# ybubnov/libhuffman

Measured on AMD Instinct MI355X. Metric: encode+decode GiB/s (uncompressed) on 64KiB blocks, higher is better.
Workload: dtype u8; 1 GPU; configs[2]: 1 GiB Zipf-distributed bytes (zipf255 seed 3), blocksize=64KiB; generator=zipf255, bytes_per_gpu=1073741824, blocksize=65536, blocks_per_gpu=16384, compressed_bytes_per_gpu=1006904592, parallelism=block-sharded x1, bit_exact_roundtrip=True, decoder=sub-index (verified), one table pass per symbol

## Files before the change

### libhuffman_amd/csrc/host/ctx.hpp

```cpp
#pragma once

#include "workspace.hpp"

struct hufgpu_ctx {
    int device;
    hipStream_t stream;
    char err[512];

    uint64_t ws_blocks;
    uint32_t *d_hist;
    hufcode_t *d_codetab;
    int16_t *d_treebuf;
    HufBlockMeta *d_meta;
    uint64_t *d_offsets;
    TwoLevel enc_sizes;
    uint64_t ws_chunks;
    uint32_t *d_chunk_hist;
    uint64_t *d_chunk_tot, *d_chunk_bits;

    uint64_t dws_blocks;
    HufDecodeMeta *d_dmeta;
    uint64_t *d_out_offsets;
    int32_t *d_status;
    TwoLevel dec_lens;
    uint32_t *d_fix_count;
    uint32_t *d_fix_blocks;
    uint32_t *d_fix_flag;

    uint64_t disc_wgs, disc_cands;
    uint32_t *d_wg_counts;
    void *d_disc_slots;
    uint64_t *d_disc_masks;
    uint64_t *d_wg_base;
    uint64_t *d_cand, *d_cand_end, *d_chain;
    int32_t *d_cand_status;
    uint32_t *d_nxt;
    uint64_t *d_walk;
    uint64_t *d_spec_off;

    uint64_t big_lanes, big_sub_bytes;
    uint64_t *d_big_entry, *d_big_exit, *d_big_pre, *d_big_wgpre, *d_big_wgscratch, *d_big_first_pos, *d_big_first_g, *d_big_last_pos;
    uint32_t *d_big_cnt;
    void *d_big_sub;
    uint64_t *d_big_offs;

    uint64_t fixed_ws;
    uint64_t *d_result;
    uint64_t complete_used, complete_raw;
    uint64_t *h_result;
    uint64_t *d_zipf;

    int profiling;
    int prof_used;
    int cur_slot;
    int n_stages;
    hipEvent_t (*ev)[MAX_STAGES + 1];
    int slot_stages[PROF_SLOTS];
    int slot_kind[PROF_SLOTS];
    int decode_pending;
    hipStream_t last_stream;
    const uint8_t *last_st;
    const uint64_t *last_offsets;
    uint8_t *last_out;
    uint64_t last_stream_len, last_out_cap, last_nblocks;
    uint64_t last_failing;
    int last_max_tree;

    uint64_t *h_bstage, *d_bstage;
    uint64_t bstage_words;
    hipEvent_t bstage_ev;
    int bstage_pending;
    uint64_t bws_blocks, bws_items;
    uint64_t *d_bprefix, *d_bobase, *d_bzero;
    uint32_t *d_blk_item;
    unsigned long long *d_item_fail;
    uint64_t *d_item_res, *h_item_res;
    uint64_t *d_bitem_offs;

    uint64_t rws_blocks, rws_ranges;
    unsigned long long *d_rcover;
    uint64_t *d_rrel, *d_rplan;
    uint32_t *d_rflag;
    unsigned long long *d_rcounters;
    unsigned long long *d_rtpairs;
    uint64_t rcounters[8];
    uint8_t *d_rscratch;
    uint64_t rscratch_bytes;

    uint64_t gws_blocks, gws_parts;
    uint32_t *d_gcnt, *d_glist;
    TwoLevel gat_scan;
    uint64_t *d_gtotal;
    void *d_gparts;
    int cus;

    uint64_t fws_words, fws_tiles, fws_edge_tiles;
    uint32_t *d_fbitmap, *d_ftcnt;
    TwoLevel find_scan;
    uint8_t *d_fedges;
    uint64_t frws_words, frws_tiles;
    uint32_t *d_frdbits, *d_frrbits, *d_frdcnt, *d_frrcnt;
    TwoLevel frec_scan;
    uint64_t *d_frdtotal;
    uint64_t fsel_ws;
    uint64_t *d_fsel_first;

    uint64_t sbws_blocks, sbws_chunks;
    uint32_t *d_sb_state;
    uint64_t *d_sb_pay, *d_sb_chunk_tot, *d_sb_chunk_bits;
    unsigned long long *d_sb_unbuilt;

    uint64_t uws_blocks, uws_pieces;
    uint32_t *d_urow_of, *d_urow_blk, *d_upiece;
    uint64_t *d_upairs, *d_unew;
    unsigned long long *d_ucount;
};

static char g_err[512] = "";

static void set_err(hufgpu_ctx *ctx, const char *fmt, ...)
{
    char buf[512];
    va_list ap;
    va_start(ap, fmt);
    vsnprintf(buf, sizeof(buf), fmt, ap);
    va_end(ap);
    snprintf(g_err, sizeof(g_err), "%s", buf);
    if (ctx) snprintf(ctx->err, sizeof(ctx->err), "%s", buf);
    fprintf(stderr, "libhuffman(gpu): %s\n", buf);
}

#define HIP_OK(ctx, call)                                                                   \
    do {                                                                                    \
        hipError_t e_ = (call);                                                             \
        if (e_ != hipSuccess) {                                                             \
            set_err((ctx), "%s failed: %s (%s:%d)", #call, hipGetErrorString(e_), __FILE__, \
                    __LINE__);                                                              \
            return HUFE_FATAL;                                                              \
        }                                                                                   \
    } while (0)


static hipError_t g_ws_error = hipSuccess;
static int ws_hip(hipError_t e)
{
    if (e == hipSuccess) return 0;
    g_ws_error = e;
    (void)hipGetLastError();
    return 1;
}
static int ws_hip_alloc_device(void **p, uint64_t bytes) { return ws_hip(hipMalloc(p, bytes)); }
static int ws_hip_alloc_pinned(void **p, uint64_t bytes) { return ws_hip(hipHostMalloc(p, bytes, hipHostMallocDefault)); }
static void ws_hip_free_device(void *p) { (void)hipFree(p); }
static void ws_hip_free_pinned(void *p) { (void)hipHostFree(p); }
static int ws_hip_zero_device(void *p, uint64_t bytes) { return ws_hip(hipMemset(p, 0, bytes)); }
static int ws_hip_wait(void) { return ws_hip(hipDeviceSynchronize()); }
static const ws_hooks WS_HIP = {ws_hip_alloc_device, ws_hip_alloc_pinned, ws_hip_free_device, ws_hip_free_pinned,
                                ws_hip_zero_device, ws_hip_wait};

#define WS_ROW(type, member, flags, expr) \
    {offsetof(type, member), [](uint64_t n, uint64_t m) -> uint64_t { (void)n; (void)m; return (expr); }, flags}
#define DEV(member, expr) WS_ROW(hufgpu_ctx, member, 0, expr)
#define DEV0(member, expr) WS_ROW(hufgpu_ctx, member, WS_ZERO, expr)
#define PIN(member, expr) WS_ROW(hufgpu_ctx, member, WS_PINNED, expr)
#define SCAN_GROUPS(n) ((n) / SCAN_GROUP + 2)

static const ws_buf WS_SCAN[] = {
    WS_ROW(TwoLevel, vals, 0, n * sizeof(uint64_t)),
    WS_ROW(TwoLevel, local, 0, n * sizeof(uint64_t)),
    WS_ROW(TwoLevel, gsum, 0, SCAN_GROUPS(n) * sizeof(uint64_t)),
    WS_ROW(TwoLevel, gprefix, 0, SCAN_GROUPS(n) * sizeof(uint64_t)),
    WS_ROW(TwoLevel, gcount, WS_ZERO, SCAN_GROUPS(n) * SCAN_TICKET_STRIDE * sizeof(uint32_t)),
    WS_ROW(TwoLevel, done, WS_ZERO, sizeof(uint32_t)),
};
static const ws_buf WS_FIXED[] = {
    DEV(d_result, 8 * sizeof(uint64_t)), PIN(h_result, 16 * sizeof(uint64_t)), DEV(d_walk, DISC_WORDS * sizeof(uint64_t)),
    DEV(d_zipf, 255 * sizeof(uint64_t)), DEV(d_big_offs, (SPEC_WORDS + 2) * sizeof(uint64_t)),
    DEV(d_rcounters, 8 * sizeof(unsigned long long)), DEV(d_gtotal, sizeof(uint64_t)),
    DEV(d_ucount, UPD_WORDS * sizeof(unsigned long long)), DEV(d_sb_unbuilt, sizeof(unsigned long long)),
};
static const ws_buf WS_ENCODE[] = {
    DEV(d_hist, n * HUF_NSYM * sizeof(uint64_t)),
    DEV(d_codetab, n * HUF_NSYM * sizeof(hufcode_t)), DEV(d_treebuf, n * HUF_TREE_STRIDE * sizeof(int16_t)),
    DEV(d_meta, n * sizeof(HufBlockMeta)), DEV(d_offsets, (n + 1) * sizeof(uint64_t)),
};
static const ws_buf WS_CHUNK[] = {
    DEV(d_chunk_hist, n * HUF_NSYM * sizeof(uint32_t)), DEV(d_chunk_tot, n * sizeof(uint64_t)), DEV(d_chunk_bits, n * sizeof(uint64_t)),
};
static const ws_buf WS_DECODE[] = {
    DEV(d_dmeta, n * sizeof(HufDecodeMeta)), DEV(d_out_offsets, (n + 1) * sizeof(uint64_t)), DEV(d_status, n * sizeof(int32_t)),
    DEV0(d_fix_count, 2 * sizeof(uint32_t)), DEV(d_fix_blocks, n * sizeof(uint32_t)), DEV0(d_fix_flag, n * sizeof(uint32_t)),
    DEV(dec_lens.gmin, SCAN_GROUPS(n) * sizeof(uint64_t)),
};
#define DISC_GCAP(n) (((n) + DISC_SCAN_GROUP - 1) / DISC_SCAN_GROUP + 1)
static const ws_buf WS_DISC_WGS[] = {
    DEV(d_wg_counts, n * sizeof(uint32_t)),
    DEV(d_wg_base, (n + 1 + 2 * DISC_GCAP(n)) * sizeof(uint64_t)),
    DEV(d_disc_masks, n * DISC_THREADS * sizeof(uint64_t)), DEV(d_disc_slots, n * DISC_SLOTS * sizeof(DiscSlot)),
};
static const ws_buf WS_DISC_CANDS[] = {
    DEV(d_cand, n * sizeof(uint64_t)), DEV(d_cand_end, n * sizeof(uint64_t)), DEV(d_chain, (n + 1) * sizeof(uint64_t)),
    DEV(d_cand_status, n * sizeof(int32_t)), DEV(d_nxt, n * sizeof(uint32_t)), DEV(d_spec_off, (n + 1) * sizeof(uint64_t)),
};
static const ws_buf WS_BIG_LANES[] = {
    DEV(d_big_entry, n * sizeof(uint64_t)), DEV(d_big_exit, n * sizeof(uint64_t)), DEV(d_big_pre, (n + 1) * sizeof(uint64_t)),
    DEV(d_big_wgpre, (n / DEC_THREADS + 4) * sizeof(uint64_t)), DEV(d_big_wgscratch, (n / DEC_THREADS + 4) * sizeof(uint64_t)),
    DEV(d_big_first_pos, n * sizeof(uint64_t)), DEV(d_big_first_g, n * sizeof(uint64_t)), DEV(d_big_last_pos, n * sizeof(uint64_t)),
    DEV(d_big_cnt, n * sizeof(uint32_t)),
};
static const ws_buf WS_BIG_SUB[] = {DEV(d_big_sub, n)};
static const ws_buf WS_BSTAGE[] = {PIN(h_bstage, n * sizeof(uint64_t)), DEV(d_bstage, n * sizeof(uint64_t))};
static const ws_buf WS_BATCH[] = {
    DEV(d_bprefix, (n + 1) * sizeof(uint64_t)), DEV(d_bobase, n * sizeof(uint64_t)), DEV0(d_bzero, SCAN_GROUPS(n) * sizeof(uint64_t)),
    DEV(d_blk_item, n * sizeof(uint32_t)), DEV(d_item_fail, m * sizeof(unsigned long long)), DEV(d_item_res, 3 * m * sizeof(uint64_t)),
    DEV(d_bitem_offs, (m + 1) * sizeof(uint64_t)), PIN(h_item_res, 3 * m * sizeof(uint64_t)),
};
static const ws_buf WS_RANGE[] = {
    DEV(d_rcover, n * sizeof(unsigned long long)), DEV(d_rrel, n * sizeof(uint64_t)), DEV(d_rtpairs, n * sizeof(unsigned long long)),
    DEV(d_rplan, 4 * m * sizeof(uint64_t)), DEV(d_rflag, m * sizeof(uint32_t)),
};
static const ws_buf WS_RSCRATCH[] = {DEV(d_rscratch, n)};
static const ws_buf WS_GATHER_BLOCKS[] = {DEV(d_gcnt, 2 * n * sizeof(uint32_t)), DEV(d_glist, n * sizeof(uint32_t))};
static const ws_buf WS_GATHER_PARTS[] = {DEV(d_gparts, n * sizeof(GatherPart))};
static const ws_buf WS_FIND_WORDS[] = {DEV(d_fbitmap, n * sizeof(uint32_t))};
static const ws_buf WS_FIND_TILES[] = {DEV(d_ftcnt, n * sizeof(uint32_t))};
static const ws_buf WS_FIND_EDGES[] = {DEV(d_fedges, n * FIND_EDGE_SLOT)};
static const ws_buf WS_FIND_REC_WORDS[] = {DEV(d_frdbits, n * sizeof(uint32_t)), DEV(d_frrbits, n * sizeof(uint32_t))};
static const ws_buf WS_FIND_REC_TILES[] = {DEV(d_frdcnt, n * sizeof(uint32_t)), DEV(d_frrcnt, n * sizeof(uint32_t)), DEV(d_frdtotal, sizeof(uint64_t))};
static const ws_buf WS_FIND_SEL[] = {DEV(d_fsel_first, n * sizeof(uint64_t))};
static const ws_buf WS_SB_BLOCKS[] = {DEV(d_sb_state, n * sizeof(uint32_t)), DEV(d_sb_pay, n * sizeof(uint64_t))};
static const ws_buf WS_SB_CHUNKS[] = {DEV(d_sb_chunk_tot, n * sizeof(uint64_t)), DEV(d_sb_chunk_bits, n * sizeof(uint64_t))};
static const ws_buf WS_UPD_BLOCKS[] = {
    DEV(d_urow_of, n * sizeof(uint32_t)), DEV(d_urow_blk, n * sizeof(uint32_t)), DEV(d_upairs, 2 * n * sizeof(uint64_t)),
    DEV(d_unew, (n + 1) * sizeof(uint64_t)),
};
static const ws_buf WS_UPD_PIECES[] = {DEV(d_upiece, n * sizeof(uint32_t))};

enum { G_FIXED, G_ENCODE, G_CHUNK, G_DECODE, G_DISC_WGS, G_DISC_CANDS, G_BIG_LANES, G_BIG_SUB, G_BSTAGE, G_BATCH, G_RANGE,
       G_RSCRATCH, G_GATHER_BLOCKS, G_GATHER_PARTS, G_FIND_WORDS, G_FIND_TILES, G_FIND_EDGES, G_FIND_REC_WORDS, G_FIND_REC_TILES, G_FIND_SEL, G_SB_BLOCKS, G_SB_CHUNKS, G_UPD_BLOCKS,
       G_UPD_PIECES, G_COUNT };
#define ROWS(a) a, (int)(sizeof(a) / sizeof(a[0]))
#define CAP(member) {offsetof(hufgpu_ctx, member), WS_NO_CAP}
#define CAPS(m0, m1) {offsetof(hufgpu_ctx, m0), offsetof(hufgpu_ctx, m1)}
#define NO_SCAN NULL, 0, 0
#define SCAN_AT(member) ROWS(WS_SCAN), offsetof(hufgpu_ctx, member)
static const ws_group WS[G_COUNT] = {
    {"fixed", ROWS(WS_FIXED), CAP(fixed_ws), WS_EXACT, false, NO_SCAN},
    {"encode", ROWS(WS_ENCODE), CAP(ws_blocks), WS_EIGHTH, false, SCAN_AT(enc_sizes)},
    {"encode chunks", ROWS(WS_CHUNK), CAP(ws_chunks), WS_EIGHTH, false, NO_SCAN},
    {"decode", ROWS(WS_DECODE), CAP(dws_blocks), WS_EIGHTH, false, SCAN_AT(dec_lens)},
    {"discovery workgroups", ROWS(WS_DISC_WGS), CAP(disc_wgs), WS_EIGHTH, false, NO_SCAN},
    {"discovery candidates", ROWS(WS_DISC_CANDS), CAP(disc_cands), WS_EIGHTH, false, NO_SCAN},
    {"big-block lanes", ROWS(WS_BIG_LANES), CAP(big_lanes), WS_EIGHTH, true, NO_SCAN},
    {"big-block sub-index", ROWS(WS_BIG_SUB), CAP(big_sub_bytes), WS_EXACT, true, NO_SCAN},
    {"batch staging", ROWS(WS_BSTAGE), CAP(bstage_words), WS_QUARTER, false, NO_SCAN},
    {"batch", ROWS(WS_BATCH), CAPS(bws_blocks, bws_items), WS_EIGHTH, false, NO_SCAN},
    {"ranges", ROWS(WS_RANGE), CAPS(rws_blocks, rws_ranges), WS_EIGHTH, false, NO_SCAN},
    {"range scratch", ROWS(WS_RSCRATCH), CAP(rscratch_bytes), WS_EXACT, true, NO_SCAN},
    {"gather blocks", ROWS(WS_GATHER_BLOCKS), CAP(gws_blocks), WS_DOUBLE, false, SCAN_AT(gat_scan)},
    {"gather parts", ROWS(WS_GATHER_PARTS), CAP(gws_parts), WS_DOUBLE, false, NO_SCAN},
    {"find words", ROWS(WS_FIND_WORDS), CAP(fws_words), WS_DOUBLE, false, NO_SCAN},
    {"find tiles", ROWS(WS_FIND_TILES), CAP(fws_tiles), WS_DOUBLE, false, SCAN_AT(find_scan)},
    {"find edges", ROWS(WS_FIND_EDGES), CAP(fws_edge_tiles), WS_DOUBLE, false, NO_SCAN},
    {"find record words", ROWS(WS_FIND_REC_WORDS), CAP(frws_words), WS_DOUBLE, false, NO_SCAN},
    {"find record tiles", ROWS(WS_FIND_REC_TILES), CAP(frws_tiles), WS_DOUBLE, false, SCAN_AT(frec_scan)},
    {"find select", ROWS(WS_FIND_SEL), CAP(fsel_ws), WS_EXACT, false, NO_SCAN},
    {"sub-build blocks", ROWS(WS_SB_BLOCKS), CAP(sbws_blocks), WS_EIGHTH, false, NO_SCAN},
    {"sub-build chunks", ROWS(WS_SB_CHUNKS), CAP(sbws_chunks), WS_EIGHTH, false, NO_SCAN},
    {"update blocks", ROWS(WS_UPD_BLOCKS), CAP(uws_blocks), WS_EIGHTH, false, NO_SCAN},
    {"update pieces", ROWS(WS_UPD_PIECES), CAP(uws_pieces), WS_EIGHTH, false, NO_SCAN},
};

static int grow_ws(hufgpu_ctx *c, int group, uint64_t need0, uint64_t need1 = 0)
{
    if (ws_grow(&WS_HIP, c, &WS[group], need0, need1) == 0) return HUFE_OK;
    if (WS[group].soft) return HUFE_MEMORY;
    set_err(c, "no workspace for %s (%llu, %llu): %s", WS[group].name, (unsigned long long)need0, (unsigned long long)need1,
            hipGetErrorString(g_ws_error));
    return HUFE_FATAL;
}
static int grow_ws2(hufgpu_ctx *c, int g0, uint64_t need0, int g1, uint64_t need1)
{
    const int rc = grow_ws(c, g0, need0);
    return rc ? rc : grow_ws(c, g1, need1);
}

static int ensure_encode_ws(hufgpu_ctx *c, uint64_t nblocks)
{
    const bool grows = nblocks > c->ws_blocks;
    const int rc = grow_ws(c, G_ENCODE, nblocks);
    if (grows) ws_release(&WS_HIP, c, &WS[G_CHUNK]);
    return rc;
}
static int ensure_chunk_ws(hufgpu_ctx *c, uint64_t nchunks) { return grow_ws(c, G_CHUNK, nchunks); }
static int ensure_decode_ws(hufgpu_ctx *c, uint64_t nblocks) { return grow_ws(c, G_DECODE, nblocks); }
static int ensure_batch_ws(hufgpu_ctx *c, uint64_t nblocks, uint64_t nitems) { return grow_ws(c, G_BATCH, nblocks, nitems); }
static int ensure_range_ws(hufgpu_ctx *c, uint64_t nblocks, uint64_t nranges) { return grow_ws(c, G_RANGE, nblocks, nranges); }
static int ensure_gather_ws(hufgpu_ctx *c, uint64_t nblocks, uint64_t nparts) { return grow_ws2(c, G_GATHER_BLOCKS, nblocks, G_GATHER_PARTS, nparts); }
static int ensure_find_ws(hufgpu_ctx *c, uint64_t nwords, uint64_t ntiles) { return grow_ws2(c, G_FIND_WORDS, nwords, G_FIND_TILES, ntiles); }
static int ensure_update_ws(hufgpu_ctx *c, uint64_t nblocks, uint64_t npieces) { return grow_ws2(c, G_UPD_BLOCKS, nblocks, G_UPD_PIECES, npieces); }
static int ensure_sub_build_ws(hufgpu_ctx *c, uint64_t nblocks, uint64_t nchunks) { return grow_ws2(c, G_SB_BLOCKS, nblocks, G_SB_CHUNKS, nchunks); }

static int grow_range_scratch(hufgpu_ctx *ctx, uint64_t bytes)
{
    if (bytes <= ctx->rscratch_bytes) return HUFE_OK;
    if (bytes > ((uint64_t)1 << 46)) {
        (void)ws_hip_wait();
        ws_release(&WS_HIP, ctx, &WS[G_RSCRATCH]);
        return HUFE_MEMORY;
    }
    if (grow_ws(ctx, G_RSCRATCH, bytes + bytes / 8) == HUFE_OK) return HUFE_OK;
    return grow_ws(ctx, G_RSCRATCH, bytes);
}

static void free_batch_stage(hufgpu_ctx *c)
{
    if (c->bstage_pending) (void)hipEventSynchronize(c->bstage_ev);
    ws_release(&WS_HIP, c, &WS[G_BSTAGE]);
    c->bstage_pending = 0;
}

extern "C" int hufgpu_device_count(void)
{
    int n = 0;
    if (hipGetDeviceCount(&n) != hipSuccess) {
        (void)hipGetLastError();
        return 0;
    }
    int usable = 0;
    for (int d = 0; d < n; d++) {
        hipDeviceProp_t p;
        if (hipGetDeviceProperties(&p, d) == hipSuccess && strncmp(p.gcnArchName, "gfx950", 6) == 0) usable++;
    }
    return usable;
}

extern "C" const char *hufgpu_last_error(const hufgpu_ctx_t *ctx) { return ctx ? ctx->err : g_err; }

static int ctx_init(hufgpu_ctx *ctx)
{
    HIP_OK(NULL, hipSetDevice(ctx->device));
    const int rc = grow_ws(ctx, G_FIXED, 1);
    if (rc) return rc;
    uint64_t cum[255], acc = 0;
    for (int r = 1; r <= 255; r++) {
        acc += (1ull << 32) / (uint64_t)r;
        cum[r - 1] = acc;
    }
    HIP_OK(ctx, hipMemcpy(ctx->d_zipf, cum, sizeof(cum), hipMemcpyHostToDevice));
    return HUFE_OK;
}

extern "C" int hufgpu_ctx_create(hufgpu_ctx_t **out, int device)
{
    if (!out) return HUFE_ARGUMENT;
    *out = NULL;
    int n = 0;
    hipError_t e = hipGetDeviceCount(&n);
    if (e != hipSuccess || n <= 0) {
        (void)hipGetLastError();
        set_err(NULL, "no HIP device available (%s); this library has no CPU fallback",
                e != hipSuccess ? hipGetErrorString(e) : "0 devices");
        return HUFE_FATAL;
    }
    if (device < 0 || device >= n) {
        set_err(NULL, "device %d out of range (have %d)", device, n);
        return HUFE_ARGUMENT;
    }
    hipDeviceProp_t prop;
    HIP_OK(NULL, hipGetDeviceProperties(&prop, device));
    if (strncmp(prop.gcnArchName, "gfx950", 6) != 0) {
        set_err(NULL, "device %d is %s; the kernels are built for gfx950 only", device, prop.gcnArchName);
        return HUFE_FATAL;
    }
    hufgpu_ctx *ctx = (hufgpu_ctx *)calloc(1, sizeof(hufgpu_ctx));
    if (!ctx) return HUFE_MEMORY;
    ctx->device = device;
    ctx->cus = prop.multiProcessorCount > 0 ? prop.multiProcessorCount : 256;
    const int rc = ctx_init(ctx);
    if (rc) {
        (void)hufgpu_ctx_destroy(ctx);
        return rc;
    }
    *out = ctx;
    return HUFE_OK;
}

extern "C" int hufgpu_ctx_device(const hufgpu_ctx_t *ctx) { return ctx ? ctx->device : -1; }

extern "C" int hufgpu_ctx_destroy(hufgpu_ctx_t *ctx)
{
    if (!ctx) return HUFE_ARGUMENT;
    (void)hipSetDevice(ctx->device);
    (void)ws_hip_wait();
    free_batch_stage(ctx);
    if (ctx->bstage_ev) (void)hipEventDestroy(ctx->bstage_ev);
    ws_release_all(&WS_HIP, ctx, WS, G_COUNT);
    if (ctx->ev) {
        for (int k = 0; k < PROF_SLOTS; k++)
            for (int i = 0; i <= MAX_STAGES; i++) (void)hipEventDestroy(ctx->ev[k][i]);
        free(ctx->ev);
    }
    free(ctx);
    return HUFE_OK;
}

static inline hipStream_t pick_stream(hufgpu_ctx *c, void *stream) { (void)c; return (hipStream_t)stream; }
static inline unsigned grid256(uint64_t n) { return (unsigned)((n + 255) / 256); }
```

### libhuffman_amd/csrc/kernels/tree.hpp

```cpp
#pragma once
#include <hip/hip_runtime.h>
#include <stdint.h>

#include "../hufgpu_common.h"
#include "util.hpp"

namespace hufgpu {

template <typename K, typename H = uint32_t>
__global__ __launch_bounds__(64) void tree_kernel(const H *__restrict__ hist, uint64_t n,
                                                  uint64_t blocksize, hufcode_t *__restrict__ codetab,
                                                  int16_t *__restrict__ treebuf,
                                                  HufBlockMeta *__restrict__ meta)
{
    __shared__ int16_t s_left[HUF_NSLOT];
    __shared__ int16_t s_right[HUF_NSLOT];
    __shared__ uint16_t s_leaves[HUF_NSLOT];
    __shared__ uint16_t s_depth[HUF_NSLOT];
    __shared__ uint16_t s_pos[HUF_NSLOT];
    __shared__ uint64_t s_code[HUF_NSLOT];
    __shared__ int16_t s_tree[HUF_TREE_STRIDE];

    const K KMAX = ~(K)0;
    const int lane = lane_id();
    const uint64_t blk = blockIdx.x;
    const H *h = hist + blk * HUF_NSYM;

    K key[8];
    H rate[4];
#pragma unroll
    for (int j = 0; j < 4; j++) {
        const int slot = lane + 64 * j;
        rate[j] = h[slot];
        key[j] = rate[j] ? (((K)rate[j] << 9) | (K)(511 - slot)) : KMAX;
    }
#pragma unroll
    for (int j = 4; j < 8; j++) key[j] = KMAX;
#pragma unroll
    for (int j = 0; j < 8; j++) {
        const int slot = lane + 64 * j;
        s_left[slot] = -1;
        s_right[slot] = -1;
        s_leaves[slot] = (j < 4 && rate[j & 3]) ? 1 : 0;
        s_depth[slot] = 0xffffu;
    }
    __syncthreads();

    int node = HUF_NSYM;
    int root = -1;
    for (;;) {
        K a = KMAX, b = KMAX;
#pragma unroll
        for (int j = 0; j < 8; j++) {
            const K k = key[j];
            const K t = dmax(a, k);
            a = dmin(a, k);
            b = dmin(b, t);
        }
#pragma unroll
        for (int o = 1; o < 64; o <<= 1) {
            const K oa = shfl_xor_key(a, o);
            const K ob = shfl_xor_key(b, o);
            const K t = dmax(a, oa);
            a = dmin(a, oa);
            b = dmin(dmin(b, ob), t);
        }
        if (a == KMAX) {
            root = node - 1;
            break;
        }
        const int i1 = 511 - (int)(a & (K)511);
        if (b == KMAX) {
            if (lane == 0) {
                s_left[node] = (int16_t)i1;
                s_right[node] = -1;
                s_leaves[node] = s_leaves[i1];
            }
            root = node;
            node++;
            break;
        }
        const int i2 = 511 - (int)(b & (K)511);
        const K sum = (a >> 9) + (b >> 9);
        const K nk = (sum << 9) | (K)(511 - node);
#pragma unroll
        for (int j = 0; j < 8; j++) {
            const int slot = lane + 64 * j;
            if (slot == i1 || slot == i2) key[j] = KMAX;
            if (slot == node) key[j] = nk;
        }
        if (lane == 0) {
            s_left[node] = (int16_t)i1;
            s_right[node] = (int16_t)i2;
            s_leaves[node] = (uint16_t)(s_leaves[i1] + s_leaves[i2]);
        }
        node++;
    }
    __syncthreads();

    const int nodes = node;
    const int nleaves = (root >= 0) ? (int)s_leaves[root] : 0;
    const int tree_len = (root >= 0) ? 4 * nleaves + 1 : 1;

    for (int i = lane; i < HUF_TREE_STRIDE; i += 64) s_tree[i] = -1;
    if (lane == 0 && root >= 0) {
        s_depth[root] = 0;
        s_code[root] = 0;
        s_pos[root] = 0;
    }
    __syncthreads();

    for (int d = 0; d < HUF_NSLOT; d++) {
        bool any = false;
#pragma unroll
        for (int j = 4; j < 8; j++) {
            const int slot = lane + 64 * j;
            if (slot < nodes && s_depth[slot] == (uint16_t)d) {
                any = true;
                const int l = s_left[slot], r = s_right[slot];
                const uint64_t c = s_code[slot];
                const int p = s_pos[slot];
                s_tree[p] = (int16_t)slot;
                s_depth[l] = (uint16_t)(d + 1);
                s_code[l] = c << 1;
                s_pos[l] = (uint16_t)(p + 1);
                if (l < HUF_NSYM) s_tree[p + 1] = (int16_t)l;
                if (r >= 0) {
                    const int pr = p + 1 + 4 * (int)s_leaves[l] - 1;
                    s_depth[r] = (uint16_t)(d + 1);
                    s_code[r] = (c << 1) | 1u;
                    s_pos[r] = (uint16_t)pr;
                    if (r < HUF_NSYM) s_tree[pr] = (int16_t)r;
                }
            }
        }
        __syncthreads();
        if (!__any(any)) break;
    }

    uint64_t bits = 0;
    uint32_t maxlen = 0;
#pragma unroll
    for (int j = 0; j < 4; j++) {
        const int slot = lane + 64 * j;
        hufcode_t e = 0;
        if (rate[j]) {
            const uint32_t len = s_depth[slot];
            e = (s_code[slot] << 8) | (hufcode_t)len;
            bits += (uint64_t)rate[j] * len;
            maxlen = dmax(maxlen, len);
        }
        codetab[blk * HUF_NSYM + slot] = e;
    }
#pragma unroll
    for (int o = 1; o < 64; o <<= 1) {
        bits += shfl_xor_u64(bits, o);
        maxlen = dmax(maxlen, wave_xor_any(maxlen, o));
    }
    int16_t *tb = treebuf + blk * HUF_TREE_STRIDE;
    for (int i = lane; i < tree_len; i += 64) tb[i] = s_tree[i];
    if (lane == 0) {
        HufBlockMeta m;
        m.tree_len = (uint32_t)tree_len;
        m.max_len = maxlen;
        m.payload_bits = bits;
        meta[blk] = m;
    }
    (void)n;
    (void)blocksize;
}

__device__ __forceinline__ uint32_t wave_min_u32(uint32_t v)
{
    asm volatile("s_nop 1\n\t"
                 "v_min_u32_dpp %0, %0, %0 quad_perm:[1,0,3,2] row_mask:0xf bank_mask:0xf\n\t"
                 "s_nop 1\n\t"
                 "v_min_u32_dpp %0, %0, %0 quad_perm:[2,3,0,1] row_mask:0xf bank_mask:0xf\n\t"
                 "s_nop 1\n\t"
                 "v_min_u32_dpp %0, %0, %0 row_half_mirror row_mask:0xf bank_mask:0xf\n\t"
                 "s_nop 1\n\t"
                 "v_min_u32_dpp %0, %0, %0 row_mirror row_mask:0xf bank_mask:0xf\n\t"
                 "s_nop 1\n\t"
                 "v_min_u32_dpp %0, %0, %0 row_bcast:15 row_mask:0xa bank_mask:0xf\n\t"
                 "s_nop 1\n\t"
                 "v_min_u32_dpp %0, %0, %0 row_bcast:31 row_mask:0xc bank_mask:0xf\n\t"
                 "s_nop 1"
                 : "+v"(v));
    return (uint32_t)__builtin_amdgcn_readlane((int)v, 63);
}

template <int R>
__device__ __forceinline__ void wave_sort_r(uint32_t (&k)[4])
{
    const uint32_t lane = (uint32_t)lane_id();
#pragma unroll
    for (uint32_t kk = 2; kk <= 64u * R; kk <<= 1) {
#pragma unroll
        for (uint32_t jj = kk >> 1; jj >= 1; jj >>= 1) {
            if (jj >= (uint32_t)R) {
                const bool up = ((lane * (uint32_t)R) & kk) == 0u;
                const bool lower = (lane & (jj / R)) == 0u;
#pragma unroll
                for (int r = 0; r < R; r++) {
                    const uint32_t d = jj / R;
                    const uint32_t o = d == 1 ? wave_xor_u32<1>(k[r]) : d == 2 ? wave_xor_u32<2>(k[r]) : d == 4 ? wave_xor_u32<4>(k[r])
                                     : d == 8 ? wave_xor_u32<8>(k[r]) : d == 16 ? wave_xor_u32<16>(k[r]) : wave_xor_u32<32>(k[r]);
                    k[r] = (lower == up) ? dmin(k[r], o) : dmax(k[r], o);
                }
            } else {
#pragma unroll
                for (uint32_t r = 0; r < (uint32_t)R; r++) {
                    if (r & jj) continue;
                    const bool up = ((lane * (uint32_t)R + r) & kk) == 0u;
                    const uint32_t lo = dmin(k[r], k[r | jj]), hi = dmax(k[r], k[r | jj]);
                    k[r] = up ? lo : hi;
                    k[r | jj] = up ? hi : lo;
                }
            }
        }
    }
}
__device__ __forceinline__ void wave_sort256(uint32_t (&k)[4]) { wave_sort_r<4>(k); }

template <int R>
__device__ __forceinline__ void wave_merge_r(uint32_t (&k)[4])
{
    const uint32_t lane = (uint32_t)lane_id();
    constexpr int STAGES = R == 4 ? 8 : (R == 2 ? 7 : 6);
#pragma unroll
    for (int st = STAGES - 1; st >= 0; st--) {
        const uint32_t jj = 1u << st;
        if (jj >= (uint32_t)R) {
            const bool lower = (lane & (jj / R)) == 0u;
#pragma unroll
            for (int r = 0; r < R; r++) {
                const uint32_t d = jj / R;
                const uint32_t o = d == 1 ? wave_xor_u32<1>(k[r]) : d == 2 ? wave_xor_u32<2>(k[r]) : d == 4 ? wave_xor_u32<4>(k[r])
                                 : d == 8 ? wave_xor_u32<8>(k[r]) : d == 16 ? wave_xor_u32<16>(k[r]) : wave_xor_u32<32>(k[r]);
                k[r] = lower ? dmin(k[r], o) : dmax(k[r], o);
            }
        } else {
#pragma unroll
            for (uint32_t r = 0; r < (uint32_t)R; r++) {
                if (r & jj) continue;
                const uint32_t lo = dmin(k[r], k[r | jj]), hi = dmax(k[r], k[r | jj]);
                k[r] = lo;
                k[r | jj] = hi;
            }
        }
    }
}

struct TreeLds {
    uint64_t state[HUF_NSLOT];
    uint16_t lcnt[HUF_NSLOT];
};

#define TREE_ANC_ROOT 0x3ffu
__device__ __forceinline__ uint64_t tree_state(uint32_t anc, uint32_t depth, uint32_t pos, uint32_t code)
{
    return ((uint64_t)code << 32) | (uint64_t)(anc | (depth << 10) | (pos << 16));
}

#define TREE_WAVE_SYNC()                                        \
    do {                                                        \
        __builtin_amdgcn_fence(__ATOMIC_ACQ_REL, "workgroup");  \
        __builtin_amdgcn_wave_barrier();                        \
    } while (0)

#ifndef TREE_ROUND_MIN
#define TREE_ROUND_MIN 16u
#endif

#define TREE_DBG_SLOTS 36
#define TREE_DBG_BLOCKS 0
#define TREE_DBG_ONE_SYMBOL 3
#define TREE_DBG_ROUND_SORTED 4
#define TREE_DBG_ROUND_IN_ORDER 7
#define TREE_DBG_SINGLE 10
#define TREE_DBG_R_4_2 13
#define TREE_DBG_R_2_1 14
#define TREE_DBG_R_4_1 15
#define TREE_DBG_NODES_IN_ORDER 16
#define TREE_DBG_NODES_SORTED1 18
#define TREE_DBG_NODES_SORTED2 20
#define TREE_DBG_NODES_CHANCE 22
#define TREE_DBG_CHECK_PASS 23
#define TREE_DBG_CHECK_FAIL 26
#define TREE_DBG_WRAP_ROOT 29
#define TREE_DBG_PATH_ROUNDS 30
#ifdef TREE_DEBUG
__device__ unsigned long long g_tree_dbg[TREE_DBG_SLOTS];
#define TREE_DBG(i, v) do { if (lane_id() == 0) atomicAdd(&g_tree_dbg[i], (unsigned long long)(v)); } while (0)
#else
#define TREE_DBG(i, v) do { } while (0)
#endif

__device__ __forceinline__ uint64_t tree_fast_wave(const uint32_t (&rate)[4], TreeLds &L, uint64_t blk,
                                               hufcode_t *__restrict__ codetab, int16_t *__restrict__ treebuf,
                                               HufBlockMeta *__restrict__ meta)
{
    uint64_t *s_state = L.state;
    uint16_t *s_lcnt = L.lcnt;
    const uint32_t KMAX = 0xffffffffu;
    const int lane = lane_id();

    {
        const unsigned long long nz0 = __ballot(rate[0] != 0), nz1 = __ballot(rate[1] != 0);
        const unsigned long long nz2 = __ballot(rate[2] != 0), nz3 = __ballot(rate[3] != 0);
        if (__popcll(nz0) + __popcll(nz1) + __popcll(nz2) + __popcll(nz3) == 1) {
            const int j1 = nz0 ? 0 : (nz1 ? 1 : (nz2 ? 2 : 3));
            const unsigned long long m1 = nz0 | nz1 | nz2 | nz3;
            const int sym = __builtin_ctzll(m1) + 64 * j1;
            uint32_t cnt = 0;
#pragma unroll
            for (int j = 0; j < 4; j++) cnt += rate[j];
#pragma unroll
            for (int o = 1; o < 64; o <<= 1) cnt += wave_xor_any(cnt, o);
            int16_t *tb1 = treebuf + blk * HUF_TREE_STRIDE;
            if (lane < 5) tb1[lane] = (lane == 0) ? (int16_t)256 : (lane == 1 ? (int16_t)sym : (int16_t)-1);
            HufBlockMeta mm;
            mm.tree_len = 5;
            mm.max_len = 1;
            mm.payload_bits = cnt;
            if (lane == 0) meta[blk] = mm;
            TREE_DBG(TREE_DBG_ONE_SYMBOL, 1);
            return encoded_block_bytes(mm);
        }
    }

    uint32_t k[4];
#pragma unroll
    for (int j = 0; j < 4; j++) {
        const int slot = lane + 64 * j;
        k[j] = rate[j] ? ((rate[j] << 9) | (uint32_t)(511 - slot)) : KMAX;
        s_lcnt[slot] = rate[j] ? 1 : 0;
    }

    uint32_t *s_scratch = reinterpret_cast<uint32_t *>(s_state + HUF_NSYM);
    uint32_t live, R = 4;
    {
        const unsigned long long nz0 = __ballot(rate[0] != 0), nz1 = __ballot(rate[1] != 0);
        const unsigned long long nz2 = __ballot(rate[2] != 0), nz3 = __ballot(rate[3] != 0);
        const uint32_t c0 = (uint32_t)__popcll(nz0), c1 = (uint32_t)__popcll(nz1), c2 = (uint32_t)__popcll(nz2), c3 = (uint32_t)__popcll(nz3);
        live = c0 + c1 + c2 + c3;
        if (live <= 128u) {
            const unsigned long long below = (1ull << lane) - 1ull;
            if (rate[0]) s_scratch[(uint32_t)__popcll(nz0 & below)] = k[0];
            if (rate[1]) s_scratch[c0 + (uint32_t)__popcll(nz1 & below)] = k[1];
            if (rate[2]) s_scratch[c0 + c1 + (uint32_t)__popcll(nz2 & below)] = k[2];
            if (rate[3]) s_scratch[c0 + c1 + c2 + (uint32_t)__popcll(nz3 & below)] = k[3];
            TREE_WAVE_SYNC();
            R = live <= 64u ? 1u : 2u;
#pragma unroll
            for (uint32_t r = 0; r < 4; r++) {
                const uint32_t c = (uint32_t)lane * R + r;
                k[r] = (r < R && c < live) ? s_scratch[c] : KMAX;
            }
            TREE_WAVE_SYNC();
        }
    }
    TREE_DBG(TREE_DBG_BLOCKS + (R >> 1), 1);

    int node = HUF_NSYM;
    int root = -1;
    bool sorted = false;
    for (;;) {
        uint32_t a, b;
        uint32_t t[4];
        if (sorted) {
            a = wave_lane_u32(k[0], 0);
            b = R == 1u ? wave_lane_u32(k[0], 1) : wave_lane_u32(k[1], 0);
#pragma unroll
            for (int j = 0; j < 4; j++) t[j] = (k[j] == a) ? KMAX : k[j];
        } else {
            a = wave_min_u32(dmin(dmin(k[0], k[1]), dmin(k[2], k[3])));
            if (a != KMAX) {
#pragma unroll
                for (int j = 0; j < 4; j++) t[j] = (k[j] == a) ? KMAX : k[j];
                b = wave_min_u32(dmin(dmin(t[0], t[1]), dmin(t[2], t[3])));
            } else {
                b = KMAX;
#pragma unroll
                for (int j = 0; j < 4; j++) t[j] = k[j];
            }
        }
        if (a == KMAX) { root = node - 1; break; }
        const int i1 = 511 - (int)(a & 511u);
        if (b == KMAX) {
            if (lane == 0) {
                s_state[i1] = tree_state((uint32_t)node, 1u, 1u, 0u);
                s_lcnt[node] = s_lcnt[i1];
            }
            root = node;
            node++;
            TREE_DBG(TREE_DBG_WRAP_ROOT, 1);
            break;
        }
        {
            const uint32_t thr = (a >> 9) + (b >> 9);
            uint32_t sel = 0;
#pragma unroll
            for (int j = 0; j < 4; j++) sel += (uint32_t)__popcll(__ballot((k[j] >> 9) < thr));
            const uint32_t round_min = R == 4u ? TREE_ROUND_MIN : (R == 2u ? TREE_ROUND_MIN / 2u : TREE_ROUND_MIN / 4u);
            if (sel >= round_min) {
                const uint32_t pairs = sel >> 1;
                TREE_DBG((sorted ? TREE_DBG_ROUND_IN_ORDER : TREE_DBG_ROUND_SORTED) + (R >> 1), 1);
                if (R == 4u) {
                    if (!sorted) wave_sort_r<4>(k);
#pragma unroll
                    for (int h = 0; h < 2; h++) {
                        const uint32_t p = 2u * (uint32_t)lane + (uint32_t)h;
                        if (p < pairs) {
                            const uint32_t x = k[2 * h], y = k[2 * h + 1];
                            const int n = node + (int)p;
                            const int xi = 511 - (int)(x & 511u), yi = 511 - (int)(y & 511u);
                            const uint32_t lx = s_lcnt[xi];
                            s_state[xi] = tree_state((uint32_t)n, 1u, 1u, 0u);
                            s_state[yi] = tree_state((uint32_t)n, 1u, 4u * lx, 1u);
                            s_lcnt[n] = (uint16_t)(lx + s_lcnt[yi]);
                            k[2 * h] = (((x >> 9) + (y >> 9)) << 9) | (uint32_t)(511 - n);
                            k[2 * h + 1] = KMAX;
                        }
                    }
                } else if (R == 2u) {
                    if (!sorted) wave_sort_r<2>(k);
                    const uint32_t p = (uint32_t)lane;
                    if (p < pairs) {
                        const uint32_t x = k[0], y = k[1];
                        const int n = node + (int)p;
                        const int xi = 511 - (int)(x & 511u), yi = 511 - (int)(y & 511u);
                        const uint32_t lx = s_lcnt[xi];
                        s_state[xi] = tree_state((uint32_t)n, 1u, 1u, 0u);
                        s_state[yi] = tree_state((uint32_t)n, 1u, 4u * lx, 1u);
                        s_lcnt[n] = (uint16_t)(lx + s_lcnt[yi]);
                        k[0] = (((x >> 9) + (y >> 9)) << 9) | (uint32_t)(511 - n);
                        k[1] = KMAX;
                    }
                } else {
                    if (!sorted) wave_sort_r<1>(k);
                    const uint32_t p = (uint32_t)lane >> 1;
                    const uint32_t o = wave_xor_u32<1>(k[0]);
                    if (p < pairs) {
                        if ((lane & 1) == 0) {
                            const uint32_t x = k[0], y = o;
                            const int n = node + (int)p;
                            const int xi = 511 - (int)(x & 511u), yi = 511 - (int)(y & 511u);
                            const uint32_t lx = s_lcnt[xi];
                            s_state[xi] = tree_state((uint32_t)n, 1u, 1u, 0u);
                            s_state[yi] = tree_state((uint32_t)n, 1u, 4u * lx, 1u);
                            s_lcnt[n] = (uint16_t)(lx + s_lcnt[yi]);
                            k[0] = (((x >> 9) + (y >> 9)) << 9) | (uint32_t)(511 - n);
                        } else {
                            k[0] = KMAX;
                        }
                    }
                }
                node += (int)pairs;
                const uint32_t was = live;
                live -= pairs;
                const uint32_t nr = live <= 64u ? 1u : (live <= 128u ? 2u : 4u);
                s_scratch = reinterpret_cast<uint32_t *>(s_state + node);
                {
                    const uint32_t unp = live - pairs;
#pragma unroll
                    for (uint32_t r = 0; r < 4; r++) {
                        const uint32_t q = (uint32_t)lane * R + r;
                        if (r < R && q < was && k[r] != KMAX) s_scratch[q < 2u * pairs ? unp + (q >> 1) : was - 1u - q] = k[r];
                    }
                    TREE_WAVE_SYNC();
                    if (nr >= 2u) {
                        const uint32_t p0 = 2u * (uint32_t)lane, p1 = p0 + 1u;
                        uint32_t nd[4] = {KMAX, KMAX, KMAX, KMAX};
                        if (pairs <= 64u) {
                            nd[0] = (uint32_t)lane < pairs ? s_scratch[unp + (uint32_t)lane] : KMAX;
                            const uint32_t nf = (uint32_t)__builtin_amdgcn_update_dpp((int)KMAX, (int)nd[0], 0x130, 0xf, 0xf, false);
                            if (__ballot(nd[0] > nf) != 0ull) {
                                wave_sort_r<1>(nd);
                                TREE_WAVE_SYNC();
                                if ((uint32_t)lane < pairs) s_scratch[unp + (uint32_t)lane] = nd[0];
                                TREE_WAVE_SYNC();
                                TREE_DBG(TREE_DBG_NODES_SORTED1 + (nr >> 2), 1);
                            } else {
                                TREE_DBG(TREE_DBG_NODES_IN_ORDER + (nr >> 2), 1);
                            }
                        } else {
                            nd[0] = p0 < pairs ? s_scratch[unp + p0] : KMAX;
                            nd[1] = p1 < pairs ? s_scratch[unp + p1] : KMAX;
                            wave_sort_r<2>(nd);
                            TREE_WAVE_SYNC();
                            if (p0 < pairs) s_scratch[unp + p0] = nd[0];
                            if (p1 < pairs) s_scratch[unp + p1] = nd[1];
                            TREE_WAVE_SYNC();
                            TREE_DBG(TREE_DBG_NODES_SORTED2 + (nr >> 2), 1);
                        }
                    } else {
                        TREE_DBG(TREE_DBG_NODES_CHANCE, 1);
                    }
                    if (nr != R) TREE_DBG(R == 2u ? TREE_DBG_R_2_1 : (nr == 2u ? TREE_DBG_R_4_2 : TREE_DBG_R_4_1), 1);
                    R = nr;
#pragma unroll
                    for (uint32_t r = 0; r < 4; r++) {
                        const uint32_t c = (uint32_t)lane * R + r;
                        k[r] = (r < R && c < live) ? s_scratch[c] : KMAX;
                    }
                    TREE_WAVE_SYNC();
                    bool in_order;
                    if (R == 4u) {
                        wave_merge_r<4>(k);
                        const uint32_t nf = (uint32_t)__builtin_amdgcn_update_dpp((int)KMAX, (int)k[0], 0x130, 0xf, 0xf, false);
                        in_order = k[0] <= k[1] && k[1] <= k[2] && k[2] <= k[3] && k[3] <= nf;
                    } else if (R == 2u) {
                        wave_merge_r<2>(k);
                        const uint32_t nf = (uint32_t)__builtin_amdgcn_update_dpp((int)KMAX, (int)k[0], 0x130, 0xf, 0xf, false);
                        in_order = k[0] <= k[1] && k[1] <= nf;
                    } else {
                        wave_merge_r<1>(k);
                        const uint32_t nf = (uint32_t)__builtin_amdgcn_update_dpp((int)KMAX, (int)k[0], 0x130, 0xf, 0xf, false);
                        in_order = k[0] <= nf;
                    }
                    sorted = __ballot(!in_order) == 0ull;
                    TREE_DBG((sorted ? TREE_DBG_CHECK_PASS : TREE_DBG_CHECK_FAIL) + (R >> 1), 1);
                }
                continue;
            }
        }
        const int i2 = 511 - (int)(b & 511u);
        const uint32_t nk = (((a >> 9) + (b >> 9)) << 9) | (uint32_t)(511 - node);
#pragma unroll
        for (int j = 0; j < 4; j++) k[j] = (k[j] == a) ? nk : ((t[j] == b) ? KMAX : t[j]);
        sorted = false;
        TREE_DBG(TREE_DBG_SINGLE + (R >> 1), 1);
        if (lane == 0) {
            const uint32_t lx = s_lcnt[i1];
            s_state[i1] = tree_state((uint32_t)node, 1u, 1u, 0u);
            s_state[i2] = tree_state((uint32_t)node, 1u, 4u * lx, 1u);
            s_lcnt[node] = (uint16_t)(lx + s_lcnt[i2]);
        }
        node++;
        live--;
    }
    if (lane == 0 && root >= 0) s_state[root] = tree_state(TREE_ANC_ROOT, 0u, 0u, 0u);
    TREE_WAVE_SYNC();
    const int nodes = node;
    const int nleaves = (root >= 0) ? (int)s_lcnt[root] : 0;
    const int tree_len = (root >= 0) ? 4 * nleaves + 1 : 1;

    uint32_t w0[8], w1[8];
    bool have[8];
#pragma unroll
    for (int j = 0; j < 8; j++) {
        const int slot = lane + 64 * j;
        have[j] = (j < 4) ? (rate[j & 3] != 0) : (slot < nodes);
        const uint64_t st = have[j] ? s_state[slot] : tree_state(TREE_ANC_ROOT, 0u, 0u, 0u);
        w0[j] = (uint32_t)st;
        w1[j] = (uint32_t)(st >> 32);
    }
#pragma unroll 1
    for (int round = 0; round < 6; round++) {
        bool pending = false;
#pragma unroll
        for (int j = 0; j < 8; j++) {
            const uint32_t anc = w0[j] & 0x3ffu;
            if (anc != TREE_ANC_ROOT) {
                const uint64_t up = s_state[anc];
                const uint32_t u0 = (uint32_t)up, u1 = (uint32_t)(up >> 32);
                w1[j] |= u1 << ((w0[j] >> 10) & 63u);
                w0[j] = ((w0[j] & ~0x3ffu) + (u0 & ~0x3ffu)) | (u0 & 0x3ffu);
                s_state[lane + 64 * j] = ((uint64_t)w1[j] << 32) | w0[j];
                pending = pending || (u0 & 0x3ffu) != TREE_ANC_ROOT;
            }
        }
        if (!__any(pending)) {
            TREE_DBG(TREE_DBG_PATH_ROUNDS + round, 1);
            break;
        }
    }

    int16_t *tb = treebuf + blk * HUF_TREE_STRIDE;
#pragma unroll
    for (int j = 0; j < 8; j++) {
        if (have[j]) {
            const uint32_t p = w0[j] >> 16;
            tb[p] = (int16_t)(lane + 64 * j);
            if (j < 4) { tb[p + 1] = -1; tb[p + 2] = -1; }
        }
    }
    if (lane == 0 && root >= 0) tb[tree_len - 1] = -1;

    uint64_t bits = 0;
    uint32_t maxlen = 0;
#pragma unroll
    for (int j = 0; j < 4; j++) {
        const int slot = lane + 64 * j;
        hufcode_t e = 0;
        if (rate[j]) {
            const uint32_t len = (w0[j] >> 10) & 63u;
            e = ((hufcode_t)w1[j] << 8) | (hufcode_t)len;
            bits += (uint64_t)rate[j] * len;
            maxlen = dmax(maxlen, len);
        }
        codetab[blk * HUF_NSYM + slot] = e;
    }
#pragma unroll
    for (int o = 1; o < 64; o <<= 1) {
        bits += shfl_xor_u64(bits, o);
        maxlen = dmax(maxlen, wave_xor_any(maxlen, o));
    }
    HufBlockMeta mm;
    mm.tree_len = (uint32_t)tree_len;
    mm.max_len = maxlen;
    mm.payload_bits = bits;
    if (lane == 0) meta[blk] = mm;
    return encoded_block_bytes(mm);
}

}
```

### libhuffman_amd/csrc/kernels/util.hpp

```cpp
#pragma once
#include <hip/hip_runtime.h>
#include <stdint.h>

#include "../hufgpu_common.h"

namespace hufgpu {

__device__ __forceinline__ int lane_id() { return (int)(threadIdx.x & 63u); }

__device__ __forceinline__ uint32_t uni32(uint32_t v) { return (uint32_t)__builtin_amdgcn_readfirstlane((int)v); }
__device__ __forceinline__ uint64_t uni64(uint64_t v)
{
    return ((uint64_t)uni32((uint32_t)(v >> 32)) << 32) | uni32((uint32_t)v);
}
__device__ __forceinline__ void pin_uniform(uint64_t v)
{
    asm volatile("" :: "s"((uint32_t)v), "s"((uint32_t)(v >> 32)));
}

template <typename T>
__device__ __forceinline__ T dmin(T a, T b) { return a < b ? a : b; }
template <typename T>
__device__ __forceinline__ T dmax(T a, T b) { return a > b ? a : b; }

__device__ __forceinline__ uint64_t encoded_block_bytes(const HufBlockMeta &m)
{
    return (uint64_t)HUF_HEADER_FIXED + 2ull * m.tree_len + ((m.payload_bits + 7) >> 3);
}

__device__ __forceinline__ uint4 load_stream16(const uint4 *p)
{
    typedef uint32_t v4u __attribute__((ext_vector_type(4)));
    const v4u v = __builtin_nontemporal_load(reinterpret_cast<const v4u *>(p));
    return make_uint4(v.x, v.y, v.z, v.w);
}
__device__ __forceinline__ void store_stream16(uint4 *p, uint4 v)
{
    typedef uint32_t v4u __attribute__((ext_vector_type(4)));
    v4u t; t.x = v.x; t.y = v.y; t.z = v.z; t.w = v.w;
    __builtin_nontemporal_store(t, reinterpret_cast<v4u *>(p));
}
__device__ __forceinline__ void store_pack16(uint4 *p, uint4 v)
{
    *p = v;
}

__device__ __forceinline__ uint32_t wave_xor_any(uint32_t v, int o);
__device__ __forceinline__ uint64_t shfl_xor_u64(uint64_t v, int mask)
{
    return ((uint64_t)wave_xor_any((uint32_t)(v >> 32), mask) << 32) | wave_xor_any((uint32_t)v, mask);
}
__device__ __forceinline__ uint32_t shfl_xor_key(uint32_t v, int mask) { return (uint32_t)__shfl_xor((int)v, mask); }
__device__ __forceinline__ uint64_t shfl_xor_key(uint64_t v, int mask) { return shfl_xor_u64(v, mask); }

__device__ __forceinline__ uint32_t wave_incl_scan_u32(uint32_t v)
{
    v += (uint32_t)__builtin_amdgcn_update_dpp(0, (int)v, 0x111, 0xf, 0xf, true);
    v += (uint32_t)__builtin_amdgcn_update_dpp(0, (int)v, 0x112, 0xf, 0xf, true);
    v += (uint32_t)__builtin_amdgcn_update_dpp(0, (int)v, 0x114, 0xf, 0xf, true);
    v += (uint32_t)__builtin_amdgcn_update_dpp(0, (int)v, 0x118, 0xf, 0xf, true);
    v += (uint32_t)__builtin_amdgcn_update_dpp(0, (int)v, 0x142, 0xa, 0xf, false);
    v += (uint32_t)__builtin_amdgcn_update_dpp(0, (int)v, 0x143, 0xc, 0xf, false);
    return v;
}
__device__ __forceinline__ uint32_t wave_excl_max_u32(uint32_t v)
{
#define HUF_MAX_DPP_(ctrl, rmask, bc) { const uint32_t o_ = (uint32_t)__builtin_amdgcn_update_dpp(0, (int)v, ctrl, rmask, 0xf, bc); v = v > o_ ? v : o_; }
    HUF_MAX_DPP_(0x111, 0xf, true)
    HUF_MAX_DPP_(0x112, 0xf, true)
    HUF_MAX_DPP_(0x114, 0xf, true)
    HUF_MAX_DPP_(0x118, 0xf, true)
    HUF_MAX_DPP_(0x142, 0xa, false)
    HUF_MAX_DPP_(0x143, 0xc, false)
#undef HUF_MAX_DPP_
    return (uint32_t)__builtin_amdgcn_update_dpp(0, (int)v, 0x138, 0xf, 0xf, true);
}
__device__ __forceinline__ uint32_t pk_max_u16(uint32_t a, uint32_t b)
{
    typedef unsigned short us2 __attribute__((ext_vector_type(2)));
    const us2 r = __builtin_elementwise_max(__builtin_bit_cast(us2, a), __builtin_bit_cast(us2, b));
    return __builtin_bit_cast(uint32_t, r);
}

template <int D>
__device__ __forceinline__ uint32_t wave_xor_u32(uint32_t v)
{
    if constexpr (D == 1) return (uint32_t)__builtin_amdgcn_update_dpp(0, (int)v, 0xB1, 0xf, 0xf, false);
    else if constexpr (D == 2) return (uint32_t)__builtin_amdgcn_update_dpp(0, (int)v, 0x4E, 0xf, 0xf, false);
    else if constexpr (D == 4) {
        const uint32_t a = (uint32_t)__builtin_amdgcn_update_dpp(0, (int)v, 0x124, 0xf, 0xf, false);
        const uint32_t b = (uint32_t)__builtin_amdgcn_update_dpp(0, (int)v, 0x12C, 0xf, 0xf, false);
        return (lane_id() & 4) ? a : b;
    } else if constexpr (D == 8) return (uint32_t)__builtin_amdgcn_update_dpp(0, (int)v, 0x128, 0xf, 0xf, false);
    else if constexpr (D == 16) return (uint32_t)__builtin_amdgcn_ds_swizzle((int)v, 0x401F);
    else return (uint32_t)__shfl_xor((int)v, D);
}

__device__ __forceinline__ uint32_t wave_xor_any(uint32_t v, int o)
{
    return o == 1 ? wave_xor_u32<1>(v) : o == 2 ? wave_xor_u32<2>(v) : o == 4 ? wave_xor_u32<4>(v)
         : o == 8 ? wave_xor_u32<8>(v) : o == 16 ? wave_xor_u32<16>(v) : wave_xor_u32<32>(v);
}
__device__ __forceinline__ uint32_t wave_up1_u32(uint32_t v)
{
    return (uint32_t)__builtin_amdgcn_update_dpp((int)v, (int)v, 0x138, 0xf, 0xf, false);
}

__device__ __forceinline__ uint32_t wave_lane_u32(uint32_t v, uint32_t uniform_lane)
{
    return (uint32_t)__builtin_amdgcn_readlane((int)v, (int)uniform_lane);
}

__device__ __forceinline__ uint32_t wave_total_u32(uint32_t v) { return wave_lane_u32(wave_incl_scan_u32(v), 63); }

template <int THREADS>
__device__ __forceinline__ uint32_t block_excl_scan_u32(uint32_t v, uint32_t *s_part, uint32_t &total)
{
    const int lane = lane_id();
    const int wave = (int)(threadIdx.x >> 6);
    const uint32_t inc = wave_incl_scan_u32(v);
    if (lane == 63) s_part[wave] = inc;
    __syncthreads();
    uint32_t base = 0, tot = 0;
#pragma unroll
    for (int i = 0; i < THREADS / 64; i++) {
        const uint32_t x = s_part[i];
        if (i < wave) base += x;
        tot += x;
    }
    __syncthreads();
    total = tot;
    return base + inc - v;
}

template <int THREADS, typename T>
__device__ __forceinline__ T block_excl_scan(T v, T *s_part, T &total)
{
    const int lane = lane_id();
    const int wave = (int)(threadIdx.x >> 6);
    T inc = v;
#pragma unroll
    for (int o = 1; o < 64; o <<= 1) {
        T t;
        if constexpr (sizeof(T) == 8) {
            uint32_t lo = (uint32_t)inc, hi = (uint32_t)((uint64_t)inc >> 32);
            lo = (uint32_t)__shfl_up((int)lo, o);
            hi = (uint32_t)__shfl_up((int)hi, o);
            t = (T)(((uint64_t)hi << 32) | lo);
        } else {
            t = (T)__shfl_up((int)inc, o);
        }
        if (lane >= o) inc += t;
    }
    if (lane == 63) s_part[wave] = inc;
    __syncthreads();
    T base = 0, tot = 0;
#pragma unroll
    for (int i = 0; i < THREADS / 64; i++) {
        T x = s_part[i];
        if (i < wave) base += x;
        tot += x;
    }
    __syncthreads();
    total = tot;
    return base + inc - v;
}

}
```

Baseline: 849.1 GiB/s.

## Use med3 compare-exchange in wave sort and stage tree row in LDS

Bitonic sort and merge compare-exchanges now use v_med3_u32 against a lane-derived all-ones or zero bound instead of separate min/max and select. The stages that stay within a lane drop their per-lane direction test. The tree row is built in LDS, pre-filled with -1 and scattered there, then written to global memory as 16-byte vector stores instead of scattered 2-byte stores. A host allocation check enforces 16-byte alignment, and DPP moves switch from update_dpp to mov_dpp. The tree kernel is a small part of the encode and decode pipeline, so any effect on end-to-end throughput is likely small.

```diff
diff --git a/libhuffman_amd/csrc/host/ctx.hpp b/libhuffman_amd/csrc/host/ctx.hpp
--- a/libhuffman_amd/csrc/host/ctx.hpp
+++ b/libhuffman_amd/csrc/host/ctx.hpp
@@ -149,7 +149,16 @@
     (void)hipGetLastError();
     return 1;
 }
-static int ws_hip_alloc_device(void **p, uint64_t bytes) { return ws_hip(hipMalloc(p, bytes)); }
+#define WS_DEVICE_ALIGN 16u
+static int ws_hip_alloc_device(void **p, uint64_t bytes)
+{
+    if (ws_hip(hipMalloc(p, bytes))) return 1;
+    if (((uintptr_t)*p & (WS_DEVICE_ALIGN - 1u)) == 0) return 0;
+    (void)hipFree(*p);
+    *p = NULL;
+    g_ws_error = hipErrorInvalidDevicePointer;
+    return 1;
+}
 static int ws_hip_alloc_pinned(void **p, uint64_t bytes) { return ws_hip(hipHostMalloc(p, bytes, hipHostMallocDefault)); }
 static void ws_hip_free_device(void *p) { (void)hipFree(p); }
 static void ws_hip_free_pinned(void *p) { (void)hipHostFree(p); }
diff --git a/libhuffman_amd/csrc/kernels/tree.hpp b/libhuffman_amd/csrc/kernels/tree.hpp
--- a/libhuffman_amd/csrc/kernels/tree.hpp
+++ b/libhuffman_amd/csrc/kernels/tree.hpp
@@ -192,30 +192,38 @@
 template <int R>
 __device__ __forceinline__ void wave_sort_r(uint32_t (&k)[4])
 {
-    const uint32_t lane = (uint32_t)lane_id();
 #pragma unroll
     for (uint32_t kk = 2; kk <= 64u * R; kk <<= 1) {
+        const uint32_t down = kk / R;
 #pragma unroll
         for (uint32_t jj = kk >> 1; jj >= 1; jj >>= 1) {
             if (jj >= (uint32_t)R) {
-                const bool up = ((lane * (uint32_t)R) & kk) == 0u;
-                const bool lower = (lane & (jj / R)) == 0u;
+                const uint32_t bound = down >= 64u ? ones_where_lane_bit(jj / R) : xor_here_u32(ones_where_lane_bit(jj / R), ones_where_lane_bit(down));
 #pragma unroll
                 for (int r = 0; r < R; r++) {
                     const uint32_t d = jj / R;
                     const uint32_t o = d == 1 ? wave_xor_u32<1>(k[r]) : d == 2 ? wave_xor_u32<2>(k[r]) : d == 4 ? wave_xor_u32<4>(k[r])
                                      : d == 8 ? wave_xor_u32<8>(k[r]) : d == 16 ? wave_xor_u32<16>(k[r]) : wave_xor_u32<32>(k[r]);
-                    k[r] = (lower == up) ? dmin(k[r], o) : dmax(k[r], o);
+                    k[r] = med3_u32(k[r], o, bound);
                 }
-            } else {
+            } else if (kk < (uint32_t)R || down >= 64u) {
 #pragma unroll
                 for (uint32_t r = 0; r < (uint32_t)R; r++) {
                     if (r & jj) continue;
-                    const bool up = ((lane * (uint32_t)R + r) & kk) == 0u;
+                    const bool up = (r & kk) == 0u;
                     const uint32_t lo = dmin(k[r], k[r | jj]), hi = dmax(k[r], k[r | jj]);
                     k[r] = up ? lo : hi;
                     k[r | jj] = up ? hi : lo;
                 }
+            } else {
+                const uint32_t bound = ones_where_lane_bit(down), nbound = ~bound;
+#pragma unroll
+                for (uint32_t r = 0; r < (uint32_t)R; r++) {
+                    if (r & jj) continue;
+                    const uint32_t x = k[r], y = k[r | jj];
+                    k[r] = med3_u32(x, y, bound);
+                    k[r | jj] = med3_u32(x, y, nbound);
+                }
             }
         }
     }
@@ -225,19 +233,18 @@
 template <int R>
 __device__ __forceinline__ void wave_merge_r(uint32_t (&k)[4])
 {
-    const uint32_t lane = (uint32_t)lane_id();
     constexpr int STAGES = R == 4 ? 8 : (R == 2 ? 7 : 6);
 #pragma unroll
     for (int st = STAGES - 1; st >= 0; st--) {
         const uint32_t jj = 1u << st;
         if (jj >= (uint32_t)R) {
-            const bool lower = (lane & (jj / R)) == 0u;
+            const uint32_t bound = ones_where_lane_bit(jj / R);
 #pragma unroll
             for (int r = 0; r < R; r++) {
                 const uint32_t d = jj / R;
                 const uint32_t o = d == 1 ? wave_xor_u32<1>(k[r]) : d == 2 ? wave_xor_u32<2>(k[r]) : d == 4 ? wave_xor_u32<4>(k[r])
                                  : d == 8 ? wave_xor_u32<8>(k[r]) : d == 16 ? wave_xor_u32<16>(k[r]) : wave_xor_u32<32>(k[r]);
-                k[r] = lower ? dmin(k[r], o) : dmax(k[r], o);
+                k[r] = med3_u32(k[r], o, bound);
             }
         } else {
 #pragma unroll
@@ -251,10 +258,11 @@
     }
 }
 
-struct TreeLds {
+struct alignas(16) TreeLds {
     uint64_t state[HUF_NSLOT];
     uint16_t lcnt[HUF_NSLOT];
 };
+#define TREE_ROW_UNITS 129
 
 #define TREE_ANC_ROOT 0x3ffu
 __device__ __forceinline__ uint64_t tree_state(uint32_t anc, uint32_t depth, uint32_t pos, uint32_t code)
@@ -577,16 +585,29 @@
         }
     }
 
-    int16_t *tb = treebuf + blk * HUF_TREE_STRIDE;
+    static_assert(TREE_ROW_UNITS * 16 == HUF_TREE_STRIDE * sizeof(int16_t), "a treebuf row is whole 16-byte units: every row starts 16-byte aligned when the buffer does (host/ctx.hpp)");
+    static_assert(TREE_ROW_UNITS * 16 <= sizeof(L.state) && alignof(TreeLds) >= 16, "the row's image lies in TreeLds::state");
+    uint4 *s_img = reinterpret_cast<uint4 *>(s_state);
+    uint16_t *s_img16 = reinterpret_cast<uint16_t *>(s_state);
+    TREE_WAVE_SYNC();
+#pragma unroll
+    for (int i = 0; i < (TREE_ROW_UNITS + 63) / 64; i++) {
+        const int u = lane + 64 * i;
+        if (u < TREE_ROW_UNITS) s_img[u] = make_uint4(~0u, ~0u, ~0u, ~0u);
+    }
+    TREE_WAVE_SYNC();
 #pragma unroll
     for (int j = 0; j < 8; j++) {
-        if (have[j]) {
-            const uint32_t p = w0[j] >> 16;
-            tb[p] = (int16_t)(lane + 64 * j);
-            if (j < 4) { tb[p + 1] = -1; tb[p + 2] = -1; }
-        }
-    }
-    if (lane == 0 && root >= 0) tb[tree_len - 1] = -1;
+        if (have[j]) s_img16[(w0[j] >> 16) & 0x7ffu] = (uint16_t)(lane + 64 * j);
+    }
+    TREE_WAVE_SYNC();
+    uint4 *row = reinterpret_cast<uint4 *>(treebuf + blk * HUF_TREE_STRIDE);
+    const int units = dmin((2 * tree_len + 15) >> 4, TREE_ROW_UNITS);
+#pragma unroll
+    for (int i = 0; i < (TREE_ROW_UNITS + 63) / 64; i++) {
+        const int u = lane + 64 * i;
+        if (u < units) row[u] = s_img[u];
+    }
 
     uint64_t bits = 0;
     uint32_t maxlen = 0;
diff --git a/libhuffman_amd/csrc/kernels/util.hpp b/libhuffman_amd/csrc/kernels/util.hpp
--- a/libhuffman_amd/csrc/kernels/util.hpp
+++ b/libhuffman_amd/csrc/kernels/util.hpp
@@ -82,16 +82,33 @@
     return __builtin_bit_cast(uint32_t, r);
 }
 
+__device__ __forceinline__ uint32_t med3_u32(uint32_t a, uint32_t b, uint32_t c)
+{
+    uint32_t r;
+    asm("v_med3_u32 %0, %1, %2, %3" : "=v"(r) : "v"(a), "v"(b), "v"(c));
+    return r;
+}
+__device__ __forceinline__ uint32_t ones_where_lane_bit(uint32_t pow2)
+{
+    return pow2 < 64u ? (uint32_t)((int32_t)((uint32_t)lane_id() << (31 - __builtin_ctz(pow2))) >> 31) : 0u;
+}
+__device__ __forceinline__ uint32_t xor_here_u32(uint32_t a, uint32_t b)
+{
+    uint32_t r;
+    asm volatile("v_xor_b32 %0, %1, %2" : "=v"(r) : "v"(a), "v"(b));
+    return r;
+}
+
 template <int D>
 __device__ __forceinline__ uint32_t wave_xor_u32(uint32_t v)
 {
-    if constexpr (D == 1) return (uint32_t)__builtin_amdgcn_update_dpp(0, (int)v, 0xB1, 0xf, 0xf, false);
-    else if constexpr (D == 2) return (uint32_t)__builtin_amdgcn_update_dpp(0, (int)v, 0x4E, 0xf, 0xf, false);
+    if constexpr (D == 1) return (uint32_t)__builtin_amdgcn_mov_dpp((int)v, 0xB1, 0xf, 0xf, false);
+    else if constexpr (D == 2) return (uint32_t)__builtin_amdgcn_mov_dpp((int)v, 0x4E, 0xf, 0xf, false);
     else if constexpr (D == 4) {
-        const uint32_t a = (uint32_t)__builtin_amdgcn_update_dpp(0, (int)v, 0x124, 0xf, 0xf, false);
-        const uint32_t b = (uint32_t)__builtin_amdgcn_update_dpp(0, (int)v, 0x12C, 0xf, 0xf, false);
+        const uint32_t a = (uint32_t)__builtin_amdgcn_mov_dpp((int)v, 0x124, 0xf, 0xf, false);
+        const uint32_t b = (uint32_t)__builtin_amdgcn_mov_dpp((int)v, 0x12C, 0xf, 0xf, false);
         return (lane_id() & 4) ? a : b;
-    } else if constexpr (D == 8) return (uint32_t)__builtin_amdgcn_update_dpp(0, (int)v, 0x128, 0xf, 0xf, false);
+    } else if constexpr (D == 8) return (uint32_t)__builtin_amdgcn_mov_dpp((int)v, 0x128, 0xf, 0xf, false);
     else if constexpr (D == 16) return (uint32_t)__builtin_amdgcn_ds_swizzle((int)v, 0x401F);
     else return (uint32_t)__shfl_xor((int)v, D);
 }
```

New measurement: 861.5 GiB/s (median of 6 runs). About the same (+1.5%).
